# nikola3794/normal-clustering-nerf

Measured on AMD Instinct MI355X. Metric: training rays/sec (+ samples/sec), higher is better.
Workload: dtype fp32 (march/composite/losses); fp16-operand MFMA with fp32 accumulate in the field MLP; 1 GPU; configs[1]+[2]: full training step, 8192 rays/GPU, normal clustering on; rays_per_gpu=8192, global_batch=8192, grid=128, max_samples=1024, parallelism=dp1, grid_update_every_16=True

## Files before the change

### normal-clustering-nerf_amd/csrc/field.hip

```cpp
#include <algorithm>
#include <type_traits>
#include <cstring>
#include "common.h"
#include "../../include/ncnerf.h"

namespace ncn {

typedef float float4_t __attribute__((ext_vector_type(4)));
typedef short short4_t __attribute__((ext_vector_type(4)));

template <typename T> struct Mfma;
template <> struct Mfma<_Float16> {
    static constexpr bool f16 = true;
    typedef _Float16 v4 __attribute__((ext_vector_type(4)));
    typedef _Float16 v8 __attribute__((ext_vector_type(8)));
    static __device__ __forceinline__ float4_t k32(v8 a, v8 b, float4_t c) {
        return __builtin_amdgcn_mfma_f32_16x16x32_f16(a, b, c, 0, 0, 0);
    }
    static __device__ __forceinline__ float4_t k16(v4 a, v4 b, float4_t c) {
        return __builtin_amdgcn_mfma_f32_16x16x16f16(a, b, c, 0, 0, 0);
    }
};
template <> struct Mfma<__bf16> {
    static constexpr bool f16 = false;
// ... 47 lines not shown
constexpr int B_L5 = 0;
constexpr int B_L2 = 4;
constexpr int N_FRAG16 = 8;
constexpr int PACKED_HALVES = N_FRAG32 * 512 + N_FRAG16 * 256;
static_assert(PACKED_HALVES == NCN_FIELD_PACKED_HALVES, "packed size");

constexpr int W1_OFF = 0, W2_OFF = W1_OFF + 64 * 32, W3_OFF = W2_OFF + 16 * 64, W4_OFF = W3_OFF + 64 * 32,
              W5_OFF = W4_OFF + 64 * 64, W_TOTAL = W5_OFF + 16 * 64;
static_assert(W_TOTAL == NCN_FIELD_NW, "weights size");

__host__ __device__ constexpr int phi(int g, int j) { return j < 4 ? 4 * g + j : 16 + 4 * g + (j - 4); }
__host__ __device__ constexpr int psi(int g, int j) {
    return j < 4 ? 3 + 4 * g + j : ((4 * g + j - 4) < 3 ? (4 * g + j - 4) : 16 + (4 * g + j - 4));
}

__host__ __device__ constexpr int frag32_index(int f, int lane, int j) {
    const int g = lane >> 4, r = lane & 15, k = phi(g, j);
    if (f < F_L2) return W1_OFF + (16 * (f - F_L1) + r) * 32 + k;
    if (f < F_L3) return W2_OFF + r * 64 + 32 * (f - F_L2) + k;
    if (f < F_L4) return W3_OFF + (16 * (f - F_L3) + r) * 32 + psi(g, j);
    if (f < F_L5) return W4_OFF + (16 * ((f - F_L4) >> 1) + r) * 64 + 32 * ((f - F_L4) & 1) + k;
    if (f < B_L4) return W5_OFF + r * 64 + 32 * (f - F_L5) + k;
    if (f < B_L3) return W4_OFF + (32 * ((f - B_L4) & 1) + k) * 64 + 16 * ((f - B_L4) >> 1) + r;
    if (f < B_L1) return W3_OFF + (32 * (f - B_L3) + k) * 32 + 3 + r;
    return W1_OFF + (32 * ((f - B_L1) & 1) + k) * 32 + 16 * ((f - B_L1) >> 1) + r;
}
__host__ __device__ constexpr int frag16_index(int f, int lane, int j) {
    const int g = lane >> 4, r = lane & 15, k = 4 * g + j;
    return f < B_L2 ? W5_OFF + k * 64 + 16 * (f - B_L5) + r : W2_OFF + k * 64 + 16 * (f - B_L2) + r;
}
__device__ float frag32_value(const float* __restrict__ W, int f, int lane, int j) { return W[frag32_index(f, lane, j)]; }
__device__ float frag16_value(const float* __restrict__ W, int f, int lane, int j) { return W[frag16_index(f, lane, j)]; }

__global__ void pack_map_kernel(int32_t* __restrict__ src) {
    const int f = blockIdx.x, lane = threadIdx.x;
    if (f < N_FRAG32) {
        for (int j = 0; j < 8; j++) src[(f * 64 + lane) * 8 + j] = frag32_index(f, lane, j);
    } else {
        const int f16 = f - N_FRAG32;
        for (int j = 0; j < 4; j++) src[N_FRAG32 * 512 + (f16 * 64 + lane) * 4 + j] = frag16_index(f16, lane, j);
    }
}

template <typename T>
__global__ void pack_weights_kernel(const float* __restrict__ W, T* __restrict__ out) {
    const int f = blockIdx.x, lane = threadIdx.x;
    if (f < N_FRAG32) {
#pragma unroll
        for (int j = 0; j < 8; j++) out[(f * 64 + lane) * 8 + j] = (T)frag32_value(W, f, lane, j);
    } else {
        const int f16 = f - N_FRAG32;
#pragma unroll
        for (int j = 0; j < 4; j++) out[N_FRAG32 * 512 + (f16 * 64 + lane) * 4 + j] = (T)frag16_value(W, f16, lane, j);
    }
}

struct LevelTable {
    float scale[16];
    uint32_t res[16], params[16], offset[16];
};

__device__ __forceinline__ uint32_t grid_index(uint32_t params, uint32_t res, uint32_t x, uint32_t y, uint32_t z) {
    uint32_t stride = 1, index = 0;
    if (stride <= params) { index += x * stride; stride *= res; }
    if (stride <= params) { index += y * stride; stride *= res; }
    if (stride <= params) { index += z * stride; stride *= res; }
    if (params < stride) index = x ^ (y * 2654435761u) ^ (z * 805459861u);
    if ((params & (params - 1)) == 0) return index & (params - 1);
    return index < params ? index : index % params;
}

struct LevelPos {
    uint32_t px, py, pz;
    float fx, fy, fz;
};
__device__ __forceinline__ LevelPos level_pos(float scale, float x, float y, float z) {
    LevelPos p;
    float a = fmaf(scale, x, 0.5f), b = fmaf(scale, y, 0.5f), c = fmaf(scale, z, 0.5f);
    const float fa = floorf(a), fb = floorf(b), fc = floorf(c);
    p.px = (uint32_t)(int)fa; p.py = (uint32_t)(int)fb; p.pz = (uint32_t)(int)fc;
    p.fx = a - fa; p.fy = b - fb; p.fz = c - fc;
    return p;
}

__device__ __forceinline__ float2 encode_level(const float2* __restrict__ tab, const LevelTable& L, int l, float x,
                                               float y, float z) {
    const LevelPos p = level_pos(L.scale[l], x, y, z);
    const uint32_t params = L.params[l], res = L.res[l], off = L.offset[l];
    uint32_t e[8];
    if ((uint64_t)res * res * res <= params) {
        const uint32_t b0 = p.px + res * p.py + res * res * p.pz;
#pragma unroll
        for (int c = 0; c < 8; c++) {
            const uint32_t i = b0 + (c & 1) + ((c >> 1) & 1) * res + ((c >> 2) & 1) * res * res;
            e[c] = i < params ? i : i % params;
        }
    } else {
        const uint32_t hy0 = p.py * 2654435761u, hy1 = (p.py + 1) * 2654435761u;
        const uint32_t hz0 = p.pz * 805459861u, hz1 = (p.pz + 1) * 805459861u;
        const uint32_t mask = params - 1;
#pragma unroll
        for (int c = 0; c < 8; c++) e[c] = ((p.px + (c & 1)) ^ ((c & 2) ? hy1 : hy0) ^ ((c & 4) ? hz1 : hz0)) & mask;
    }
    float2 v[8];
#pragma unroll
    for (int c = 0; c < 8; c++) v[c] = tab[off + e[c]];
    const float wx[2] = {1.0f - p.fx, p.fx}, wy[2] = {1.0f - p.fy, p.fy}, wz[2] = {1.0f - p.fz, p.fz};
    float2 acc = make_float2(0.f, 0.f);
#pragma unroll
    for (int c = 0; c < 8; c++) {
        const float w = (wx[c & 1] * wy[(c >> 1) & 1]) * wz[c >> 2];
        acc.x = fmaf(w, v[c].x, acc.x);
        acc.y = fmaf(w, v[c].y, acc.y);
    }
    return acc;
}

template <int CTRL>
__device__ __forceinline__ float dppf(float v) {
    return __int_as_float(__builtin_amdgcn_update_dpp(0, __float_as_int(v), CTRL, 0xF, 0xF, false));
}
template <int CTRL>
__device__ __forceinline__ int dppi(int v) {
    return __builtin_amdgcn_update_dpp(0, v, CTRL, 0xF, 0xF, false);
}
constexpr int DPP_ROW_SL(int k) { return 0x100 + k; }
constexpr int DPP_ROW_SR(int k) { return 0x110 + k; }

template <int K>
__device__ __forceinline__ void run_sum(float& v, const int (&link)[4]) {
    const float t = dppf<DPP_ROW_SL(1 << K)>(v);
    if (link[K]) v += t;
}

template <typename T>
struct Frags {
    typedef typename Mfma<T>::v4 v4;
    typedef typename Mfma<T>::v8 v8;
    const v8* f32;
    const v4* f16;
    __device__ __forceinline__ v8 a32(int f, int lane) const { return f32[f * 64 + lane]; }
    __device__ __forceinline__ v4 a16(int f, int lane) const { return f16[f * 64 + lane]; }
};
template <typename T>
struct FragsSigma : Frags<T> {
    __device__ __forceinline__ typename Mfma<T>::v8 a32(int f, int lane) const {
        return this->f32[(f >= B_L1 ? f - (B_L1 - F_L3) : f) * 64 + lane];
    }
    __device__ __forceinline__ typename Mfma<T>::v4 a16(int f, int lane) const {
        return this->f16[(f - B_L2) * 64 + lane];
    }
};
constexpr int N_SIG32 = F_L3 + 4, N_SIG16 = 4;

template <typename T>
struct FwdState {
    typedef typename Mfma<T>::v4 v4;
    v4 x2[4];
    float4_t h;
    v4 x3h, x3d;
    v4 x4[4];
    v4 x5[4];
    float4_t out;
};

template <typename T, typename FR>
__device__ __forceinline__ void mlp_sigma(const FR& F, int lane, typename Mfma<T>::v8 e, FwdState<T>& st) {
    typedef Mfma<T> M;
    typedef typename M::v8 v8;
#pragma unroll
    for (int t = 0; t < 4; t++) st.x2[t] = relu4<T>(M::k32(F.a32(F_L1 + t, lane), e, zero4()));
    float4_t h = M::k32(F.a32(F_L2, lane), cat8<v8>(st.x2[0], st.x2[1]), zero4());
    st.h = M::k32(F.a32(F_L2 + 1, lane), cat8<v8>(st.x2[2], st.x2[3]), h);
}

template <typename T>
__device__ __forceinline__ void mlp_rgb(const Frags<T>& F, int lane, float dnx, float dny, float dnz, FwdState<T>& st) {
    typedef Mfma<T> M;
    typedef typename M::v8 v8;
    const int g = lane >> 4;
    st.x3h = cvt4<T>(st.h);
    st.x3d = cvt4<T>(float4_t{g == 0 ? dnx : 1.f, g == 0 ? dny : 1.f, g == 0 ? dnz : 1.f, 1.f});
    const v8 b3 = cat8<v8>(st.x3h, st.x3d);
#pragma unroll
    for (int t = 0; t < 4; t++) st.x4[t] = relu4<T>(M::k32(F.a32(F_L3 + t, lane), b3, zero4()));
    const v8 b4a = cat8<v8>(st.x4[0], st.x4[1]), b4b = cat8<v8>(st.x4[2], st.x4[3]);
#pragma unroll
    for (int t = 0; t < 4; t++)
        st.x5[t] = relu4<T>(M::k32(F.a32(F_L4 + 2 * t + 1, lane), b4b, M::k32(F.a32(F_L4 + 2 * t, lane), b4a, zero4())));
    const float4_t o = M::k32(F.a32(F_L5, lane), cat8<v8>(st.x5[0], st.x5[1]), zero4());
    st.out = M::k32(F.a32(F_L5 + 1, lane), cat8<v8>(st.x5[2], st.x5[3]), o);
}

__device__ __forceinline__ float sigmoidf_(float x) { return 1.0f / (1.0f + __expf(-x)); }

__device__ __forceinline__ void load_levels(LevelTable& Ls, const LevelTable& La) {
    if (threadIdx.x < 16) {
        const int l = threadIdx.x;
        Ls.scale[l] = La.scale[l];
        Ls.res[l] = La.res[l];
        Ls.params[l] = La.params[l];
        Ls.offset[l] = La.offset[l];
    }
}

constexpr int SORT_W = 4096, SORT_THREADS = 1024;
__device__ __forceinline__ uint32_t sort_spread10(uint32_t v) {
    v &= 0x3FFu;
    v = (v | (v << 16)) & 0x030000FFu;
    v = (v | (v << 8)) & 0x0300F00Fu;
    v = (v | (v << 4)) & 0x030C30C3u;
    v = (v | (v << 2)) & 0x09249249u;
    return v;
}
__device__ __forceinline__ uint32_t sort_q10(float v, float mn, float inv) {
    const float q = (v - mn) * inv * 1024.0f;
    return (uint32_t)(int)fminf(fmaxf(q, 0.0f), 1023.0f);
}
__global__ __launch_bounds__(SORT_THREADS) void sort_windows_kernel(const float* __restrict__ xyzs, int64_t n,
                                                                    const int32_t* __restrict__ n_dev, float mn,
                                                                    float inv, int32_t* __restrict__ order) {
    __shared__ unsigned long long k[SORT_W];
    if (n_dev) n = min<int64_t>(n, *n_dev);
    const int64_t base = (int64_t)blockIdx.x * SORT_W;
    if (base >= n) return;
    const int cnt = (int)min<int64_t>(SORT_W, n - base);
    for (int i = threadIdx.x; i < SORT_W; i += SORT_THREADS) {
        unsigned long long key = ~0ull;
        if (i < cnt) {
            const float* x = xyzs + 3 * (base + i);
            const uint32_t m = sort_spread10(sort_q10(x[0], mn, inv)) | (sort_spread10(sort_q10(x[1], mn, inv)) << 1) |
                               (sort_spread10(sort_q10(x[2], mn, inv)) << 2);
            key = ((unsigned long long)m << 12) | (unsigned long long)i;
        }
        k[i] = key;
    }
    __syncthreads();
    for (int size = 2; size <= SORT_W; size <<= 1) {
        for (int stride = size >> 1; stride > 0; stride >>= 1) {
            for (int t = threadIdx.x; t < SORT_W / 2; t += SORT_THREADS) {
                const int lo = 2 * t - (t & (stride - 1)), hi = lo + stride;
                const bool up = (lo & size) == 0;
                const unsigned long long a = k[lo], b = k[hi];
                if ((a > b) == up) { k[lo] = b; k[hi] = a; }
            }
            __syncthreads();
        }
    }
    for (int i = threadIdx.x; i < cnt; i += SORT_THREADS) order[base + i] = (int32_t)(base + (int64_t)(k[i] & 0xFFFull));
}

template <typename T, bool DENSITY>
__global__ __launch_bounds__(256) __attribute__((amdgpu_waves_per_eu(4))) void field_fwd_kernel(const float* __restrict__ xyzs, const float* __restrict__ dirs,
                                                        int64_t n, const int32_t* __restrict__ n_dev,
                                                        const float2* __restrict__ table, LevelTable Lt,
                                                        float xyz_min, float xyz_extent,
                                                        const typename Mfma<T>::v8* __restrict__ wpacked, int mode,
                                                        float* __restrict__ sigmas, float* __restrict__ rgbs,
                                                        typename Mfma<T>::v8* __restrict__ enc_cache,
                                                        const int32_t* __restrict__ order) {
    typedef typename Mfma<T>::v8 v8;
    __shared__ v8 Fs[N_FWD32 * 64];
    __shared__ LevelTable L;
    const int64_t n16 = (n + 15) & ~(int64_t)15;
    if (n_dev) n = min<int64_t>(n, *n_dev);
    for (int i = threadIdx.x; i < N_FWD32 * 64; i += 256) Fs[i] = wpacked[i];
    load_levels(L, Lt);
    __syncthreads();
    const int lane = threadIdx.x & 63, g = lane >> 4, r = lane & 15;
    const int64_t n_groups = (n + 15) / 16;
    const int64_t wave0 = (int64_t)blockIdx.x * 4 + (threadIdx.x >> 6);
    const int64_t n_waves = (int64_t)gridDim.x * 4;
    for (int64_t grp = wave0; grp < n_groups; grp += n_waves) {
        Frags<T> F;
        F.f32 = Fs + opaque_zero();
        F.f16 = nullptr;
        const int64_t pos = grp * 16 + r;
        const bool valid = pos < n;
        const int64_t s = valid && order ? (int64_t)order[pos] : pos;
        v8 e;
        if constexpr (DENSITY) {
            typedef T t2 __attribute__((ext_vector_type(2)));
            const t2* el = (const t2*)enc_cache + pos;
            const t2 a0 = el[(2 * g) * n16], a1 = el[(2 * g + 1) * n16];
            const t2 b0 = el[(8 + 2 * g) * n16], b1 = el[(9 + 2 * g) * n16];
            e = v8{a0[0], a0[1], a1[0], a1[1], b0[0], b0[1], b1[0], b1[1]};
        } else {
            float x = 0.f, y = 0.f, z = 0.f;
            if (valid) {
                x = (xyzs[3 * s] - xyz_min) / xyz_extent;
                y = (xyzs[3 * s + 1] - xyz_min) / xyz_extent;
                z = (xyzs[3 * s + 2] - xyz_min) / xyz_extent;
            }
            const float2 e00 = encode_level(table, L, 2 * g, x, y, z);
            const float2 e01 = encode_level(table, L, 2 * g + 1, x, y, z);
            asm volatile("; encode: levels 8+ after 0-7 %1 %2" : "+v"(x) : "v"(e00.x), "v"(e01.x));
            const float2 e10 = encode_level(table, L, 8 + 2 * g, x, y, z);
            const float2 e11 = encode_level(table, L, 9 + 2 * g, x, y, z);
            e = v8{(T)e00.x, (T)e00.y, (T)e01.x, (T)e01.y, (T)e10.x, (T)e10.y, (T)e11.x, (T)e11.y};
            if (enc_cache) enc_cache[grp * 64 + lane] = e;
        }
        FwdState<T> st;
        mlp_sigma<T>(F, lane, e, st);
        if (g == 0 && valid) sigmas[s] = __expf(st.h[0]);
        if (DENSITY || mode != 0) continue;
        float dx = 0.f, dy = 0.f, dz = 0.f;
// ... 102 lines not shown
}

__device__ __forceinline__ float lmax_upd(float m, float a, float b) {
    return (isfinite(a) && isfinite(b)) ? fmaxf(m, fmaxf(fabsf(a), fabsf(b))) : INFINITY;
}
template <int PART> constexpr int x_count() { return PART == BWD_SIGMA ? N_XFRAG - XA2 : N_XFRAG; }
template <int PART> constexpr int x_origin() { return PART == BWD_SIGMA ? XA2 : 0; }

template <typename T>
struct DinCtx {
    const T* w3d;
    const int32_t* order;
    float* out;
};
template <typename T, int PART, bool DIN = false, typename FR>
__device__ __forceinline__ void bwd_group(const FR& F, uint16_t* Xw, const BwdIn<T>& cur, int64_t grp,
                                          int64_t n, int64_t n_stride, int lane, float* __restrict__ dE_out,
                                          float (&lm)[4], float inv_S, typename Mfma<T>::v4* __restrict__ stq,
                                          float* __restrict__ sth0, const DinCtx<T>* din = nullptr) {
    typedef Mfma<T> M;
    typedef typename M::v4 v4;
    typedef typename M::v8 v8;
    const int g = lane >> 4, r = lane & 15;
    const int64_t s = grp * 16 + r;
    const bool valid = s < n;
    FwdState<T> st;
    mlp_sigma<T>(F, lane, cur.e, st);
    float4_t dh;
    if constexpr ((PART & BWD_RGB) != 0) {
    float dx = cur.dx, dy = cur.dy, dz = cur.dz;
    if (valid) {
        const float nrm = sqrtf(dx * dx + dy * dy + dz * dz);
        dx /= nrm; dy /= nrm; dz /= nrm;
    }
    mlp_rgb<T>(F, lane, dx, dy, dz, st);
    float4_t dy5 = zero4();
    if (g == 0) {
        const float s0 = sigmoidf_(st.out[0]), s1 = sigmoidf_(st.out[1]), s2 = sigmoidf_(st.out[2]);
        dy5[0] = cur.dr0 * s0 * (1.f - s0);
        dy5[1] = cur.dr1 * s1 * (1.f - s1);
        dy5[2] = cur.dr2 * s2 * (1.f - s2);
    }
    const v4 dy5h = cvt4<T>(dy5);
    x_put(Xw + XA5 * 256, lane, dy5h);
#pragma unroll
    for (int b = 0; b < 4; b++) x_put(Xw + (XB5 + b) * 256, lane, st.x5[b]);
    v4 dD4[4];
#pragma unroll
    for (int t = 0; t < 4; t++) dD4[t] = relu_mask4<T>(M::k16(F.a16(B_L5 + t, lane), dy5h, zero4()), st.x5[t]);
#pragma unroll
    for (int t = 0; t < 4; t++) {
        x_put(Xw + (XA4 + t) * 256, lane, dD4[t]);
        x_put(Xw + (XB4 + t) * 256, lane, st.x4[t]);
    }
    const v8 d4a = cat8<v8>(dD4[0], dD4[1]), d4b = cat8<v8>(dD4[2], dD4[3]);
    v4 dD3[4];
#pragma unroll
    for (int t = 0; t < 4; t++)
        dD3[t] = relu_mask4<T>(M::k32(F.a32(B_L4 + 2 * t + 1, lane), d4b, M::k32(F.a32(B_L4 + 2 * t, lane), d4a, zero4())),
                                st.x4[t]);
#pragma unroll
    for (int t = 0; t < 4; t++) x_put(Xw + (XA3 + t) * 256, lane, dD3[t]);
    x_put(Xw + XB3D * 256, lane, st.x3d);
    x_put(Xw + XB3H * 256, lane, st.x3h);
    if constexpr (DIN) {
        float gi[3] = {0.f, 0.f, 0.f};
#pragma unroll
        for (int k = 0; k < 3; k++)
#pragma unroll
            for (int t = 0; t < 4; t++) {
                const v4 w = *(const v4*)(din->w3d + k * 64 + 16 * t + 4 * g);
#pragma unroll
                for (int i = 0; i < 4; i++) gi[k] = fmaf((float)w[i], (float)dD3[t][i], gi[k]);
            }
#pragma unroll
        for (int k = 0; k < 3; k++) {
            gi[k] += __shfl_xor(gi[k], 16);
            gi[k] += __shfl_xor(gi[k], 32);
        }
        if (g == 0 && valid) {
#pragma unroll
            for (int k = 0; k < 3; k++) gi[k] = (float)(T)gi[k] * inv_S;
            const float nrm = sqrtf(cur.dx * cur.dx + cur.dy * cur.dy + cur.dz * cur.dz);
            const float nx = cur.dx / nrm, ny = cur.dy / nrm, nz = cur.dz / nrm;
            const float ng = nx * gi[0] + ny * gi[1] + nz * gi[2];
            float* o = din->out + 3 * (din->order ? (int64_t)din->order[s] : s);
            o[0] = (gi[0] - nx * ng) / nrm;
            o[1] = (gi[1] - ny * ng) / nrm;
            o[2] = (gi[2] - nz * ng) / nrm;
        }
    }
    dh = M::k32(F.a32(B_L3, lane), cat8<v8>(dD3[0], dD3[1]), zero4());
    dh = M::k32(F.a32(B_L3 + 1, lane), cat8<v8>(dD3[2], dD3[3]), dh);
    if constexpr (PART == BWD_RGB) {
        stq[grp * 64 + lane] = cvt4<T>(dh);
        if (g == 0) sth0[grp * 16 + r] = dh[0];
        return;
    }
    }
    v4 dhh;
    const float tex = __expf(fminf(fmaxf(st.h[0], -15.f), 15.f));
    if constexpr (PART == BWD_SIGMA) {
        dhh = cur.dq;
        if (g == 0) dhh[0] = (T)fmaf(cur.dsig, tex, cur.h0);
    } else {
        dhh = cvt4<T>(dh);
        if (g == 0) dhh[0] = (T)fmaf(cur.dsig, tex, dh[0]);
    }
    constexpr int XO = x_origin<PART>();
    x_put(Xw + (XA2 - XO) * 256, lane, dhh);
#pragma unroll
    for (int b = 0; b < 4; b++) x_put(Xw + (XB2 - XO + b) * 256, lane, st.x2[b]);
    v4 dD1[4];
#pragma unroll
    for (int t = 0; t < 4; t++) dD1[t] = relu_mask4<T>(M::k16(F.a16(B_L2 + t, lane), dhh, zero4()), st.x2[t]);
#pragma unroll
    for (int t = 0; t < 4; t++) x_put(Xw + (XA1 - XO + t) * 256, lane, dD1[t]);
    const v4 e0 = v4{cur.e[0], cur.e[1], cur.e[2], cur.e[3]}, e1 = v4{cur.e[4], cur.e[5], cur.e[6], cur.e[7]};
    x_put(Xw + (XB1 - XO) * 256, lane, e0);
    x_put(Xw + (XB1 - XO + 1) * 256, lane, e1);
    const v8 d1a = cat8<v8>(dD1[0], dD1[1]), d1b = cat8<v8>(dD1[2], dD1[3]);
    float4_t dE[2];
#pragma unroll
    for (int t = 0; t < 2; t++)
        dE[t] = M::k32(F.a32(B_L1 + 2 * t + 1, lane), d1b, M::k32(F.a32(B_L1 + 2 * t, lane), d1a, zero4()));
    typedef T t2 __attribute__((ext_vector_type(2)));
    const t2 q[4] = {t2{(T)dE[0][0], (T)dE[0][1]}, t2{(T)dE[0][2], (T)dE[0][3]}, t2{(T)dE[1][0], (T)dE[1][1]},
                     t2{(T)dE[1][2], (T)dE[1][3]}};
#pragma unroll
    for (int j = 0; j < 4; j++) lm[j] = lmax_upd(lm[j], (float)q[j][0] * inv_S, (float)q[j][1] * inv_S);
    if (valid) {
        t2* o = (t2*)dE_out;
        o[(int64_t)(2 * g) * n_stride + s] = q[0];
        o[(int64_t)(2 * g + 1) * n_stride + s] = q[1];
        o[(int64_t)(8 + 2 * g) * n_stride + s] = q[2];
        o[(int64_t)(9 + 2 * g) * n_stride + s] = q[3];
    }
}

template <typename T, int NX = N_XFRAG, int XO = 0>
__device__ __forceinline__ typename Mfma<T>::v8 x_pair(const uint16_t* X, int q, int ng, int tile, int lane) {
    typedef typename Mfma<T>::v4 v4;
    const v4 a = x_get<v4>(X + (q * NX + tile - XO) * 256, lane);
    const v4 b = q + 1 < ng ? x_get<v4>(X + ((q + 1) * NX + tile - XO) * 256, lane) : v4{0, 0, 0, 0};
    return cat8<typename Mfma<T>::v8>(a, b);
}
template <typename T, int PART>
__device__ __forceinline__ void bwd_dw(const uint16_t* X, int ng, int wid, int lane, float4_t (&acc)[5]) {
    typedef Mfma<T> M;
    typedef typename M::v8 v8;
    constexpr bool RGB = (PART & BWD_RGB) != 0, SIG = (PART & BWD_SIGMA) != 0;
    if constexpr (PART == BWD_SIGMA) {
        constexpr int NX = x_count<PART>(), XO = x_origin<PART>();
        for (int q = 0; q < ng; q += 2) {
            acc[0] = M::k32(x_pair<T, NX, XO>(X, q, ng, XA1 + (wid >> 1), lane),
                            x_pair<T, NX, XO>(X, q, ng, XB1 + (wid & 1), lane), acc[0]);
            if (wid < 4)
                acc[1] = M::k32(x_pair<T, NX, XO>(X, q, ng, XA2, lane), x_pair<T, NX, XO>(X, q, ng, XB2 + wid, lane),
                                acc[1]);
        }
        return;
    }
    if constexpr (PART == BWD_RGB) {
        for (int q = 0; q < ng; q += 2) {
            if (wid < 4) {
                const v8 A4 = x_pair<T>(X, q, ng, XA4 + wid, lane);
#pragma unroll
                for (int b = 0; b < 4; b++) acc[b] = M::k32(A4, x_pair<T>(X, q, ng, XB4 + b, lane), acc[b]);
            } else {
                const v8 A3 = x_pair<T>(X, q, ng, XA3 + wid - 4, lane);
                acc[0] = M::k32(A3, x_pair<T>(X, q, ng, XB3D, lane), acc[0]);
                acc[1] = M::k32(A3, x_pair<T>(X, q, ng, XB3H, lane), acc[1]);
                acc[4] = M::k32(x_pair<T>(X, q, ng, XA5, lane), x_pair<T>(X, q, ng, XB5 + wid - 4, lane), acc[4]);
            }
        }
        return;
    }
    for (int q = 0; q < ng; q += 2) {
        if (wid < 4) {
            if constexpr (RGB) {
                const v8 A4 = x_pair<T>(X, q, ng, XA4 + wid, lane);
#pragma unroll
                for (int b = 0; b < 4; b++) acc[b] = M::k32(A4, x_pair<T>(X, q, ng, XB4 + b, lane), acc[b]);
                acc[4] = M::k32(x_pair<T>(X, q, ng, XA5, lane), x_pair<T>(X, q, ng, XB5 + wid, lane), acc[4]);
            }
        } else if (wid < 6) {
            if constexpr (RGB) {
                const v8 Bd = x_pair<T>(X, q, ng, XB3D, lane), Bh = x_pair<T>(X, q, ng, XB3H, lane);
#pragma unroll
                for (int aa = 0; aa < 2; aa++) {
                    const v8 A3 = x_pair<T>(X, q, ng, XA3 + 2 * (wid - 4) + aa, lane);
                    acc[2 * aa] = M::k32(A3, Bd, acc[2 * aa]);
                    acc[2 * aa + 1] = M::k32(A3, Bh, acc[2 * aa + 1]);
                }
            }
            if constexpr (SIG)
                acc[4] = M::k32(x_pair<T>(X, q, ng, XA2, lane), x_pair<T>(X, q, ng, XB2 + wid - 4, lane), acc[4]);
        } else {
            if constexpr (SIG) {
                const v8 B0 = x_pair<T>(X, q, ng, XB1, lane), B1 = x_pair<T>(X, q, ng, XB1 + 1, lane);
#pragma unroll
                for (int aa = 0; aa < 2; aa++) {
                    const v8 A1 = x_pair<T>(X, q, ng, XA1 + 2 * (wid - 6) + aa, lane);
                    acc[2 * aa] = M::k32(A1, B0, acc[2 * aa]);
                    acc[2 * aa + 1] = M::k32(A1, B1, acc[2 * aa + 1]);
                }
                acc[4] = M::k32(x_pair<T>(X, q, ng, XA2, lane), x_pair<T>(X, q, ng, XB2 + wid - 4, lane), acc[4]);
            }
        }
    }
}

template <int PART>
__device__ __forceinline__ void bwd_store_dw(float* __restrict__ out, int wid, int lane, float4_t (&acc)[5], float inv_S) {
    constexpr bool RGB = (PART & BWD_RGB) != 0, SIG = (PART & BWD_SIGMA) != 0;
    const int g = lane >> 4, r = lane & 15;
#pragma unroll
    for (int t = 0; t < 5; t++)
#pragma unroll
        for (int i = 0; i < 4; i++) acc[t][i] *= inv_S;
    if constexpr (PART == BWD_SIGMA) {
#pragma unroll
        for (int i = 0; i < 4; i++) {
            const int row = 4 * g + i;
            out[W1_OFF + (16 * (wid >> 1) + row) * 32 + 16 * (wid & 1) + r] = acc[0][i];
            if (wid < 4) out[W2_OFF + row * 64 + 16 * wid + r] = acc[1][i];
        }
        return;
    }
    if constexpr (PART == BWD_RGB) {
#pragma unroll
        for (int i = 0; i < 4; i++) {
            const int row = 4 * g + i;
            if (wid < 4) {
#pragma unroll
                for (int b = 0; b < 4; b++) out[W4_OFF + (16 * wid + row) * 64 + 16 * b + r] = acc[b][i];
            } else {
                const int orow = 16 * (wid - 4) + row;
                out[W3_OFF + orow * 32 + (r < 3 ? r : 16 + r)] = acc[0][i];
                out[W3_OFF + orow * 32 + 3 + r] = acc[1][i];
                out[W5_OFF + row * 64 + 16 * (wid - 4) + r] = acc[4][i];
            }
        }
        return;
    }
#pragma unroll
    for (int i = 0; i < 4; i++) {
        const int row = 4 * g + i;
        if (wid < 4) {
            if constexpr (RGB) {
#pragma unroll
                for (int b = 0; b < 4; b++) out[W4_OFF + (16 * wid + row) * 64 + 16 * b + r] = acc[b][i];
                out[W5_OFF + row * 64 + 16 * wid + r] = acc[4][i];
            }
        } else if (wid < 6) {
            if constexpr (RGB) {
#pragma unroll
                for (int aa = 0; aa < 2; aa++) {
                    const int orow = 16 * (2 * (wid - 4) + aa) + row;
                    out[W3_OFF + orow * 32 + (r < 3 ? r : 16 + r)] = acc[2 * aa][i];
                    out[W3_OFF + orow * 32 + 3 + r] = acc[2 * aa + 1][i];
                }
            }
            if constexpr (SIG) out[W2_OFF + row * 64 + 16 * (wid - 4) + r] = acc[4][i];
        } else {
            if constexpr (SIG) {
#pragma unroll
                for (int aa = 0; aa < 2; aa++) {
                    const int orow = 16 * (2 * (wid - 6) + aa) + row;
                    out[W1_OFF + orow * 32 + r] = acc[2 * aa][i];
                    out[W1_OFF + orow * 32 + 16 + r] = acc[2 * aa + 1][i];
                }
                out[W2_OFF + row * 64 + 16 * (wid - 4) + r] = acc[4][i];
            }
        }
    }
}

__host__ __device__ inline int bwd_blocks_of(int64_t n) {
    const int64_t groups = (n + 15) / 16;
    const int64_t b = (groups + 31) / 32;
    return (int)(b < 1 ? 1 : (b > 256 ? 256 : b));
}

template <typename T, int PART = BWD_ALL, bool DIN = false>
__global__ __launch_bounds__(BWD_THREADS) void field_bwd_kernel(
    const float* __restrict__ dirs, int64_t n, const int32_t* __restrict__ n_dev, const uint16_t* __restrict__ wpacked,
    const typename Mfma<T>::v8* __restrict__ enc_cache, const float* __restrict__ dL_dsig,
    const float* __restrict__ dL_drgb, const float* __restrict__ loss_scale, float* __restrict__ dE_out,
    float* __restrict__ slab, float* __restrict__ level_max, const int32_t* __restrict__ order,
    const float* __restrict__ dL_dsig2 = nullptr, float* __restrict__ stash = nullptr,
    const float* __restrict__ xyzs = nullptr, const float* __restrict__ w_master = nullptr,
    float* __restrict__ dL_ddirs = nullptr) {
    static_assert(!DIN || PART == BWD_ALL, "the direction gradient leaves the one-pass form only");
    typedef typename Mfma<T>::v4 v4;
    const float S = loss_scale ? *loss_scale * (Mfma<T>::f16 ? NCN_TCNN_LOSS_SCALE : 1.f) : 1.f, inv_S = 1.f / S;
    typedef typename Mfma<T>::v8 v8;
    const int64_t n_stride = (n + 3) & ~(int64_t)3;
    float* const dE_pairs = dE_out ? dE_out + DE_HEADER_FLOATS : nullptr;
    if (PART != BWD_RGB && dE_out && blockIdx.x == 0 && threadIdx.x < SC_QUEUE_WORDS) {
        if (threadIdx.x == 0) {
            dE_out[0] = inv_S;
            dE_out[1] = Mfma<T>::f16 ? 0.f : 1.f;
        }
        ((unsigned*)(dE_out + de_queue_offset(n_stride)))[threadIdx.x] = 0u;
    }
    const float* pos_src = ((PART & DE_POS_PART) != 0 && dE_out && !order) ? xyzs : nullptr;
    float* const pos_out = pos_src ? dE_out + DE_HEADER_FLOATS + 16 * n_stride : nullptr;
    const int64_t pos_stride = sc_perm_stride(n_stride);
    if ((PART & DE_POS_PART) != 0 && dE_out && blockIdx.x == 0 && threadIdx.x == 0)
        dE_out[DE_POS_FLAG] = pos_out ? (float)((1 << DE_POS_MLP_CLASSES) - 1) : 0.f;
    const int lm_rows = bwd_blocks_of(n);
    v4* stq = (v4*)stash;
    float* sth0 = stash ? stash + ((n + 15) / 16) * 128 : nullptr;
    const int64_t n_cap = n;
    if (n_dev) n = min<int64_t>(n, *n_dev);
    constexpr bool SIGONLY = PART == BWD_SIGMA;
    constexpr int NF32 = SIGONLY ? N_SIG32 : N_FRAG32, NF16 = SIGONLY ? N_SIG16 : N_FRAG16, NX = x_count<PART>();
    __shared__ v8 F32s[NF32 * 64];
    __shared__ v4 F16s[NF16 * 64];
    __shared__ __attribute__((aligned(16))) uint16_t X[BWD_WAVES * NX * 256];
    {
        const v8* w32 = (const v8*)wpacked;
        const v4* w16 = (const v4*)(wpacked + N_FRAG32 * 512);
        for (int i = threadIdx.x; i < NF32 * 64; i += BWD_THREADS) {
            const int f = i >> 6;
            F32s[i] = w32[(SIGONLY && f >= F_L3 ? f + (B_L1 - F_L3) : f) * 64 + (i & 63)];
        }
        for (int i = threadIdx.x; i < NF16 * 64; i += BWD_THREADS) F16s[i] = w16[(SIGONLY ? B_L2 * 64 : 0) + i];
    }
    if constexpr (PART == BWD_RGB) {
        if (blockIdx.x == 0 && level_max)
            for (int i = threadIdx.x; i < lm_rows * 16; i += BWD_THREADS) level_max[i] = 0.f;
    }
    DinCtx<T> din = {nullptr, order, dL_ddirs};
    if constexpr (DIN) {
        __shared__ __attribute__((aligned(16))) T W3d[3 * 64];
        for (int i = threadIdx.x; i < 3 * 64; i += BWD_THREADS) W3d[i] = (T)w_master[W3_OFF + (i & 63) * 32 + (i >> 6)];
        din.w3d = W3d;
        for (int64_t i = 3 * n + (int64_t)blockIdx.x * BWD_THREADS + threadIdx.x; i < 3 * n_cap;
             i += (int64_t)gridDim.x * BWD_THREADS)
            dL_ddirs[i] = 0.f;
    }
    __syncthreads();
    const int lane = threadIdx.x & 63, wid = threadIdx.x >> 6;
    float4_t acc[5];
#pragma unroll
    for (int t = 0; t < 5; t++) acc[t] = zero4();
    float lm[4] = {0.f, 0.f, 0.f, 0.f};
    const int64_t n_groups = (n + 15) / 16;
    const int64_t stride = (int64_t)gridDim.x * BWD_WAVES;
    int64_t base = (int64_t)blockIdx.x * BWD_WAVES;
    BwdIn<T> nxt;
    if (base + wid < n_groups)
        bwd_load<T, PART>(nxt, base + wid, n, lane, enc_cache, dirs, dL_dsig, dL_dsig2, dL_drgb, stq, sth0, order, S,
                          pos_src);
    for (; base < n_groups; base += stride) {
        const int64_t grp = base + wid;
        const int ng = (int)min<int64_t>(BWD_WAVES, n_groups - base);
        const BwdIn<T> cur = nxt;
        if (grp + stride < n_groups)
            bwd_load<T, PART>(nxt, grp + stride, n, lane, enc_cache, dirs, dL_dsig, dL_dsig2, dL_drgb, stq, sth0, order,
                              S, pos_src);
        if (grp < n_groups) {
            if ((PART & DE_POS_PART) != 0 && pos_out && (lane >> 4) < DE_POS_MLP_CLASSES && grp * 16 + (lane & 15) < n) {
                const int cls = lane >> 4;
                float* po = pos_out + cls * 3 * pos_stride + 3 * sc_perm(grp * 16 + (lane & 15), cls);
                po[0] = cur.px; po[1] = cur.py; po[2] = cur.pz;
            }
            typename std::conditional<SIGONLY, FragsSigma<T>, Frags<T>>::type F;
            const int z = opaque_zero();
            F.f32 = F32s + z;
            F.f16 = F16s + z;
            bwd_group<T, PART, DIN>(F, X + wid * NX * 256, cur, grp, n, n_stride, lane, dE_pairs, lm, inv_S, stq, sth0,
                                    &din);
        }
        lds_barrier();
        if constexpr (DIN) {
            bwd_dw<T, PART>(X, __builtin_amdgcn_readfirstlane(ng), __builtin_amdgcn_readfirstlane(wid), lane, acc);
        } else
            bwd_dw<T, PART>(X, ng, wid, lane, acc);
        lds_barrier();
    }
    bwd_store_dw<PART>(slab + (int64_t)blockIdx.x * NCN_FIELD_NW, wid, lane, acc, inv_S);
    if constexpr (PART == BWD_RGB) return;
#pragma unroll
    for (int i = 0; i < 4; i++) {
        float m = lm[i];
        m = fmaxf(m, dppf<0x128>(m));
        m = fmaxf(m, dppf<0x124>(m));
        m = fmaxf(m, dppf<0x122>(m));
        m = fmaxf(m, dppf<0x121>(m));
        lm[i] = m;
    }
    __shared__ float lmw[BWD_WAVES][16];
    if ((lane & 15) == 0) {
        const int g = lane >> 4;
        lmw[wid][2 * g] = lm[0];
        lmw[wid][2 * g + 1] = lm[1];
        lmw[wid][8 + 2 * g] = lm[2];
        lmw[wid][9 + 2 * g] = lm[3];
    }
    __syncthreads();
    if (threadIdx.x < 16) {
        float m = 0.f;
#pragma unroll
        for (int w = 0; w < BWD_WAVES; w++) m = fmaxf(m, lmw[w][threadIdx.x]);
        if constexpr (PART == BWD_SIGMA)
            atomicMax((unsigned*)&level_max[(blockIdx.x % lm_rows) * 16 + threadIdx.x], __float_as_uint(m));
        else
            level_max[blockIdx.x * 16 + threadIdx.x] = m;
    }
    if (PART == BWD_ALL && blockIdx.x == 0)
        for (int i = (int)gridDim.x * 16 + threadIdx.x; i < lm_rows * 16; i += BWD_THREADS) level_max[i] = 0.f;
}

constexpr int WRED_CHUNK = 16;
__global__ void reduce_wgrad_kernel(const float* __restrict__ slab, int nb_sigma, int nb_rgb, float* __restrict__ gw) {
    const int i = blockIdx.x * 256 + threadIdx.x;
    if (i >= NCN_FIELD_NW) return;
    const int nb = i < W3_OFF ? nb_sigma : nb_rgb;
    const int b0 = blockIdx.y * WRED_CHUNK, b1 = min(nb, b0 + WRED_CHUNK);
    if (b0 >= b1) return;
    float s = 0.f;
    for (int b = b0; b < b1; b++) s += slab[(int64_t)b * NCN_FIELD_NW + i];
    atomicAdd(gw + i, s);
}

constexpr int SC_THREADS = 1024;
constexpr int SC_WAVES = SC_THREADS / 64;
constexpr int SC_WAYS = 4;
constexpr int SC_SLOT_BYTES = 4 + 8 + 8 + 2;
constexpr int SC_SETS_DIR = 1536;
constexpr int SC_CELL_HI = 10;
constexpr int SC_CELL_VALS = 16;
constexpr int SC_SETS_CELL = 160;
constexpr int SC_QUEUE = 64;
constexpr int SC_CELL_TABLE_BYTES = SC_SETS_CELL * SC_WAYS * (4 + SC_CELL_VALS * 8 + 2);
constexpr int SC_QUEUE_BYTES = SC_WAVES * SC_QUEUE * (4 + SC_CELL_VALS * 4);
constexpr int sc_max(int a, int b) { return a > b ? a : b; }
constexpr int SC_ARENA = sc_max(SC_CELL_TABLE_BYTES + SC_QUEUE_BYTES, SC_SETS_DIR * SC_WAYS * SC_SLOT_BYTES);
static_assert(SC_CELL_TABLE_BYTES % 16 == 0, "run queues 16-B aligned");
constexpr uint32_t SC_EMPTY = 0xFFFFFFFFu;
constexpr int SC_BATCH = 2;
__host__ __device__ constexpr int sc_fine_c(int l) { return l < 15 ? 4 : 2; }
#ifndef NCN_SC_C_CELL
#define NCN_SC_C_CELL 4
#endif
constexpr int SC_C_CELL = NCN_SC_C_CELL;

__device__ __forceinline__ uint32_t sc_set(uint32_t e, uint32_t sets) { return __umulhi(e * 0x9E3779B1u, sets); }

__device__ __forceinline__ long long sc_fix(float v, int k) {
    const double magic = 6755399441055744.0;
    const double y = fma((double)v, __longlong_as_double((long long)(1023 + k) << 52), magic);
    return __double_as_longlong(y) - __double_as_longlong(magic);
}

struct ScShared {
    uint32_t* keys;
    long long *valx, *valy;
    uint16_t* used;
    float4* qval;
    uint32_t* qkey;
    uint32_t sets;
    int slots;
    int* fill;
    int* grab;
};
enum { SC_MODE_DIR = 0, SC_MODE_CELL = 1 };
__device__ __forceinline__ ScShared sc_layout(char* arena, int* fill, int mode) {
    ScShared sh;
    sh.sets = mode == SC_MODE_CELL ? SC_SETS_CELL : SC_SETS_DIR;
    sh.slots = (int)sh.sets * SC_WAYS;
    sh.valx = (long long*)arena;
    sh.valy = mode == SC_MODE_CELL ? sh.valx + (SC_CELL_VALS - 1) * sh.slots : sh.valx + sh.slots;
    sh.keys = (uint32_t*)(sh.valy + sh.slots);
    sh.used = (uint16_t*)(sh.keys + sh.slots);
    sh.qval = (float4*)(arena + SC_CELL_TABLE_BYTES);
    sh.qkey = (uint32_t*)(sh.qval + SC_WAVES * SC_QUEUE * 4);
    sh.fill = fill;
    return sh;
}

struct ScLevel {
    float scale;
    uint32_t res, params, off;
    bool dense, direct;
    int k;
};

__device__ __forceinline__ void sc_corner_entries(const ScLevel& L, uint32_t px, uint32_t py, uint32_t pz,
                                                  uint32_t (&e)[8]) {
    if (L.dense) {
        const uint32_t b0 = px + L.res * py + L.res * L.res * pz;
#pragma unroll
        for (int c = 0; c < 8; c++) {
            e[c] = b0 + (c & 1) + ((c >> 1) & 1) * L.res + ((c >> 2) & 1) * L.res * L.res;
            e[c] = e[c] < L.params ? e[c] : e[c] % L.params;
        }
    } else {
        const uint32_t hy0 = py * 2654435761u, hy1 = (py + 1) * 2654435761u;
        const uint32_t hz0 = pz * 805459861u, hz1 = (pz + 1) * 805459861u;
#pragma unroll
        for (int c = 0; c < 8; c++)
            e[c] = ((px + (c & 1)) ^ ((c & 2) ? hy1 : hy0) ^ ((c & 4) ? hz1 : hz0)) & (L.params - 1);
    }
}

__device__ __forceinline__ void sc_add(ScShared& sh, int lane, uint32_t px, uint32_t py, uint32_t pz,
                                       const float (&v)[16], const ScLevel& L, float* __restrict__ grad) {
    uint32_t e[8];
    sc_corner_entries(L, px, py, pz, e);
    if (L.direct) {
#pragma unroll
        for (int c = 0; c < 8; c++) {
            if (v[2 * c] != 0.f || v[2 * c + 1] != 0.f) {
                atomicAdd(grad + 2 * (size_t)(L.off + e[c]), v[2 * c]);
                atomicAdd(grad + 2 * (size_t)(L.off + e[c]) + 1, v[2 * c + 1]);
            }
        }
        return;
    }
    uint32_t newmask = 0;
    int slot[8];
#pragma unroll
    for (int c0 = 0; c0 < 8; c0 += SC_BATCH) {
        uint4 kk[SC_BATCH];
        int p0[SC_BATCH];
#pragma unroll
        for (int b = 0; b < SC_BATCH; b++) {
            p0[b] = SC_WAYS * sc_set(e[c0 + b], sh.sets);
            kk[b] = *(const uint4*)&sh.keys[p0[b]];
        }
        int sl[SC_BATCH];
        bool vc[SC_BATCH], miss = false;
#pragma unroll
        for (int b = 0; b < SC_BATCH; b++) {
            const uint32_t k = e[c0 + b];
            vc[b] = (v[2 * (c0 + b)] != 0.f) | (v[2 * (c0 + b) + 1] != 0.f);
            sl[b] = kk[b].x == k ? p0[b] : kk[b].y == k ? p0[b] + 1 : kk[b].z == k ? p0[b] + 2
                  : kk[b].w == k ? p0[b] + 3 : -1;
            miss |= vc[b] && sl[b] < 0;
        }
        if (__ballot(miss)) {
#pragma unroll
            for (int b = 0; b < SC_BATCH; b++) {
                if (vc[b] && sl[b] < 0) {
                    const uint32_t k = e[c0 + b];
#pragma unroll
                    for (int attempt = 0; attempt < 2 && sl[b] < 0; attempt++) {
                        if (attempt) {
                            asm volatile("" ::: "memory");
                            kk[b] = *(const uint4*)&sh.keys[p0[b]];
                        }
                        sl[b] = kk[b].x == k ? p0[b] : kk[b].y == k ? p0[b] + 1 : kk[b].z == k ? p0[b] + 2
                              : kk[b].w == k ? p0[b] + 3 : -1;
                        if (sl[b] >= 0) break;
                        const int cl = kk[b].x == SC_EMPTY ? p0[b] : kk[b].y == SC_EMPTY ? p0[b] + 1
                                     : kk[b].z == SC_EMPTY ? p0[b] + 2 : kk[b].w == SC_EMPTY ? p0[b] + 3 : -1;
                        if (cl < 0) break;
                        const uint32_t got = atomicCAS(&sh.keys[cl], SC_EMPTY, k);
                        if (got == SC_EMPTY) { sl[b] = cl; newmask |= 1u << (c0 + b); }
                        else if (got == k) sl[b] = cl;
                    }
                }
            }
// ... 923 lines not shown
    NCN_LAUNCH_CHECK("ncn_field_bwd_mlp");
    return 0;
}

int ncn_field_bwd_mlp_din(const float* xyzs, const float* dirs, int64_t n, const int32_t* n_dev, const int32_t* order,
                          const uint16_t* weights_packed, int precision, const uint16_t* enc_cache,
                          const float* dL_dsigmas, const float* dL_drgbs, const float* loss_scale, float* slab,
                          float* dE_ws, float* level_max, const float* w_master, float* dL_ddirs, void* stream) {
    if (n <= 0) return 0;
    NCN_REQUIRE(precision == NCN_PREC_F16 || precision == NCN_PREC_BF16, hipErrorInvalidValue,
                "ncn_field_bwd_mlp_din: precision must be NCN_PREC_F16 or NCN_PREC_BF16");
    NCN_REQUIRE(dirs != nullptr, hipErrorInvalidValue,
                "ncn_field_bwd_mlp_din: no direction gradient without dirs (density mode)");
    NCN_REQUIRE(w_master != nullptr && dL_ddirs != nullptr, hipErrorInvalidValue,
                "ncn_field_bwd_mlp_din: w_master and dL_ddirs required");
    NCN_REQUIRE(((uintptr_t)dE_ws & 15) == 0 && ((uintptr_t)enc_cache & 15) == 0 && ((uintptr_t)weights_packed & 15) == 0,
                hipErrorInvalidValue, "ncn_field_bwd_mlp_din: dE_ws / enc_cache / weights_packed must be 16-byte aligned");
    NCN_REQUIRE(level_max != nullptr, hipErrorInvalidValue, "ncn_field_bwd_mlp_din: level_max workspace required");
    NCN_REQUIRE(((uintptr_t)xyzs & 15) == 0, hipErrorInvalidValue, "ncn_field_bwd_mlp_din: xyzs must be 16-byte aligned");
    const int nb = ncn_field_bwd_blocks(n);
    const hipStream_t st = (hipStream_t)stream;
    if (precision == NCN_PREC_F16)
        hipLaunchKernelGGL((field_bwd_kernel<_Float16, BWD_ALL, true>), dim3(nb), dim3(BWD_THREADS), 0, st, dirs, n, n_dev,
                           weights_packed, (const Mfma<_Float16>::v8*)enc_cache, dL_dsigmas, dL_drgbs, loss_scale, dE_ws,
                           slab, level_max, order, (const float*)nullptr, (float*)nullptr, xyzs, w_master, dL_ddirs);
    else
        hipLaunchKernelGGL((field_bwd_kernel<__bf16, BWD_ALL, true>), dim3(nb), dim3(BWD_THREADS), 0, st, dirs, n, n_dev,
                           weights_packed, (const Mfma<__bf16>::v8*)enc_cache, dL_dsigmas, dL_drgbs, loss_scale, dE_ws,
                           slab, level_max, order, (const float*)nullptr, (float*)nullptr, xyzs, w_master, dL_ddirs);
    NCN_LAUNCH_CHECK("ncn_field_bwd_mlp_din");
    return 0;
}

int ncn_field_bwd_dx(const float* xyzs, int64_t n, const int32_t* n_dev, const int32_t* order, const float* table,
                     const uint32_t* levels, float xyz_min, float xyz_extent, const float* dE_ws, float* dL_dxyzs,
                     void* stream) {
    if (n <= 0) return 0;
    NCN_REQUIRE(xyzs && table && levels && dE_ws && dL_dxyzs, hipErrorInvalidValue,
                "ncn_field_bwd_dx: xyzs, table, levels, dE_ws and dL_dxyzs required");
    NCN_REQUIRE(xyz_extent > 0.f, hipErrorInvalidValue, "ncn_field_bwd_dx: xyz_extent must be positive");
    NCN_REQUIRE(((uintptr_t)table & 7) == 0 && ((uintptr_t)dE_ws & 15) == 0, hipErrorInvalidValue,
                "ncn_field_bwd_dx: table 8-byte, dE_ws 16-byte aligned");
    const LevelTable Lt = make_table(levels);
    hipLaunchKernelGGL(field_bwd_dx_kernel, dim3(fwd_grid(n)), dim3(256), 0, (hipStream_t)stream, xyzs, n, n_dev, order,
                       (const float2*)table, Lt, xyz_min, xyz_extent, dE_ws, dL_dxyzs);
    NCN_LAUNCH_CHECK("ncn_field_bwd_dx");
    return 0;
}

int64_t ncn_field_bwd_stash_floats(int64_t n) { return n > 0 ? 144 * ((n + 15) / 16) : 0; }

int ncn_field_bwd_part_blocks(int64_t n, int part) {
    const int nb = ncn_field_bwd_blocks(n);
    return part == 2 ? std::min(512, 2 * nb) : nb;
}

int ncn_field_bwd_mlp_part(const float* xyzs, const float* dirs, int64_t n, const int32_t* n_dev, const int32_t* order,
                           const uint16_t* weights_packed, int precision, const uint16_t* enc_cache,
                           const float* dL_dsigmas, const float* dL_dsigmas2, const float* dL_drgbs,
                           const float* loss_scale, int part, int n_blocks, float* slab, float* dE_ws,
                           float* level_max, float* dh_stash, void* stream) {
    if (n <= 0) return 0;
    NCN_REQUIRE(precision == NCN_PREC_F16 || precision == NCN_PREC_BF16, hipErrorInvalidValue,
                "ncn_field_bwd_mlp_part: precision must be NCN_PREC_F16 or NCN_PREC_BF16");
    NCN_REQUIRE(part == 1 || part == 2 || part == 3, hipErrorInvalidValue,
                "ncn_field_bwd_mlp_part: part must be 1 (rgb), 2 (sigma) or 3 (both)");
    NCN_REQUIRE(((uintptr_t)dE_ws & 15) == 0 && ((uintptr_t)enc_cache & 15) == 0 &&
                    ((uintptr_t)weights_packed & 15) == 0 && ((uintptr_t)dh_stash & 15) == 0,
                hipErrorInvalidValue, "ncn_field_bwd_mlp_part: dE_ws / enc_cache / weights_packed / dh_stash must be 16-byte aligned");
    NCN_REQUIRE(level_max != nullptr, hipErrorInvalidValue, "ncn_field_bwd_mlp_part: level_max workspace required");
    NCN_REQUIRE(part == 3 || dh_stash != nullptr, hipErrorInvalidValue, "ncn_field_bwd_mlp_part: dh_stash required for a split pass");
    const int nb = n_blocks > 0 ? std::min(n_blocks, ncn_field_bwd_part_blocks(n, part))
                                : ncn_field_bwd_part_blocks(n, part);
    const hipStream_t st = (hipStream_t)stream;
    if (part == 1)
        launch_bwd_part<1>(precision, nb, st, xyzs, dirs, n, n_dev, weights_packed, enc_cache, dL_dsigmas, dL_drgbs,
                           loss_scale, dE_ws, slab, level_max, order, dL_dsigmas2, dh_stash);
    else if (part == 2)
        launch_bwd_part<2>(precision, nb, st, xyzs, dirs, n, n_dev, weights_packed, enc_cache, dL_dsigmas, dL_drgbs,
                           loss_scale, dE_ws, slab, level_max, order, dL_dsigmas2, dh_stash);
    else
        launch_bwd_part<3>(precision, nb, st, xyzs, dirs, n, n_dev, weights_packed, enc_cache, dL_dsigmas, dL_drgbs,
                           loss_scale, dE_ws, slab, level_max, order, dL_dsigmas2, dh_stash);
    NCN_LAUNCH_CHECK("ncn_field_bwd_mlp_part");
    return 0;
}

int ncn_field_scatter_wgrad(const float* xyzs, int64_t n, const int32_t* n_dev, const int32_t* order,
                            const uint32_t* levels, float xyz_min, float xyz_extent, const float* dE_ws,
                            const float* level_max, int level_lo, int level_hi, int max_blocks, float* grad_table,
                            const float* slab, int n_blocks_sigma, int n_blocks_rgb, float* grad_w, void* stream) {
    if (n <= 0 || level_hi <= level_lo) return slab ? ncn_field_reduce_wgrad_parts(slab, n_blocks_sigma, n_blocks_rgb,
                                                                                   grad_w, stream) : 0;
    NCN_REQUIRE(0 <= level_lo && level_hi <= 16, hipErrorInvalidValue, "ncn_field_scatter: levels must lie in [0, 16)");
    NCN_REQUIRE(((uintptr_t)dE_ws & 15) == 0 && ((uintptr_t)xyzs & 15) == 0, hipErrorInvalidValue,
                "ncn_field_scatter: dE_ws and xyzs must be 16-byte aligned");
    NCN_REQUIRE(!slab || grad_w, hipErrorInvalidValue, "ncn_field_scatter_wgrad: grad_w required with a slab");
    const LevelTable Lt = make_table(levels);
    int grid = scatter_grid(n);
    if (max_blocks > 0) grid = std::min(grid, max_blocks * (1024 / SC_THREADS));
    hipLaunchKernelGGL(field_scatter_kernel, dim3(grid), dim3(SC_THREADS), 0, (hipStream_t)stream, xyzs, n, n_dev, Lt,
                       xyz_min, xyz_extent, dE_ws, grad_table, level_max, ncn_field_bwd_blocks(n),
                       level_lo, level_hi, order, slab, n_blocks_sigma, n_blocks_rgb, grad_w,
                       (unsigned*)const_cast<float*>(dE_ws + de_queue_offset((n + 3) & ~(int64_t)3)) + 2 * level_lo);
    NCN_LAUNCH_CHECK("ncn_field_scatter");
    return 0;
}

int ncn_field_scatter_positions(const float* xyzs, int64_t n, const int32_t* n_dev, float* dE_ws, void* stream) {
    if (n <= 0) return 0;
    NCN_REQUIRE(((uintptr_t)dE_ws & 15) == 0 && ((uintptr_t)xyzs & 15) == 0, hipErrorInvalidValue,
                "ncn_field_scatter_positions: dE_ws and xyzs must be 16-byte aligned");
    const int64_t e_stride = (n + 3) & ~(int64_t)3;
    const int pgrid = (int)std::max<int64_t>(1, std::min<int64_t>(1024, cdiv(cdiv(n, 4), 256)));
    hipLaunchKernelGGL(sc_perm_positions_kernel, dim3(pgrid), dim3(256), 0, (hipStream_t)stream, xyzs, n, n_dev,
                       (1 << SC_N_CLASSES) - 1, dE_ws + DE_HEADER_FLOATS + 16 * e_stride, dE_ws + DE_POS_FLAG,
                       (float)((1 << SC_N_CLASSES) - 1));
    NCN_LAUNCH_CHECK("ncn_field_scatter_positions");
    return 0;
}

int ncn_field_scatter(const float* xyzs, int64_t n, const int32_t* n_dev, const int32_t* order,
                      const uint32_t* levels, float xyz_min,
                      float xyz_extent, const float* dE_ws, const float* level_max, int level_lo, int level_hi,
                      int max_blocks, float* grad_table, void* stream) {
    return ncn_field_scatter_wgrad(xyzs, n, n_dev, order, levels, xyz_min, xyz_extent, dE_ws, level_max, level_lo,
                                   level_hi, max_blocks, grad_table, nullptr, 0, 0, nullptr, stream);
}

int ncn_field_bwd(const float* xyzs, const float* dirs, int64_t n, const int32_t* n_dev, const int32_t* order,
                  const uint32_t* levels,
                  float xyz_min, float xyz_extent, const uint16_t* weights_packed, int precision,
                  const uint16_t* enc_cache, const float* dL_dsigmas, const float* dL_drgbs, const float* loss_scale,
                  float* grad_table, float* slab, float* dE_ws, float* level_max, void* stream) {
    if (n <= 0) return 0;
    const int e = ncn_field_bwd_mlp(xyzs, dirs, n, n_dev, order, weights_packed, precision, enc_cache, dL_dsigmas, dL_drgbs,
                                    loss_scale, slab, dE_ws, level_max, stream);
    if (e) return e;
    return ncn_field_scatter(xyzs, n, n_dev, order, levels, xyz_min, xyz_extent, dE_ws, level_max, 0, 16, 0,
                             grad_table, stream);
}


#ifdef NCN_DIAG_SC_TIMES
int ncn_diag_sc_times(unsigned long long* host, int reset) {
    if (reset) {
        static unsigned long long zero[256][10];
        return (int)hipMemcpyToSymbol(HIP_SYMBOL(ncn_sc_times), zero, sizeof(zero));
    }
    return (int)hipMemcpyFromSymbol(host, HIP_SYMBOL(ncn_sc_times), 256 * 10 * sizeof(unsigned long long));
}
#endif

#ifdef NCN_DIAG_SC_SPAN
int ncn_diag_sc_span(unsigned long long* host) {
    return (int)hipMemcpyFromSymbol(host, HIP_SYMBOL(ncn_sc_span), 256 * 20 * sizeof(unsigned long long));
}
#endif

int ncn_field_reduce_wgrad(const float* slab, int n_blocks, float* grad_w, void* stream) {
    if (n_blocks <= 0) return 0;
    hipLaunchKernelGGL(reduce_wgrad_kernel, dim3(cdiv(NCN_FIELD_NW, 256), cdiv(n_blocks, WRED_CHUNK)), dim3(256), 0,
                       (hipStream_t)stream, slab, n_blocks, n_blocks, grad_w);
    NCN_LAUNCH_CHECK("ncn_field_reduce_wgrad");
    return 0;
}

int ncn_field_reduce_wgrad_parts(const float* slab, int n_blocks_sigma, int n_blocks_rgb, float* grad_w,
                                 void* stream) {
    const int nb = std::max(n_blocks_sigma, n_blocks_rgb);
    if (nb <= 0) return 0;
    hipLaunchKernelGGL(reduce_wgrad_kernel, dim3(cdiv(NCN_FIELD_NW, 256), cdiv(nb, WRED_CHUNK)), dim3(256), 0,
                       (hipStream_t)stream, slab, n_blocks_sigma, n_blocks_rgb, grad_w);
    NCN_LAUNCH_CHECK("ncn_field_reduce_wgrad_parts");
    return 0;
}

}
```

Before: 11.46 million rays/s.

## Hold sigma-only backward weight fragments in registers and overlap first load

The sigma-only backward kernel now copies most of its MFMA weight fragments from LDS into registers once per block, instead of reading them from LDS on every group. It issues the first group's input load before the weight staging and barrier, fully unrolls the weight-gradient loop when a block has a full set of groups, and sets a higher minimum waves-per-EU launch bound for the sigma part. Cycle-counter probes are added behind a diagnostic macro that is off by default. The extra register use competes with the occupancy hint and could cause spills.

Result: faster. 11.70 million rays/s (median of 6 runs) (+2.1%).

```diff
diff --git a/normal-clustering-nerf_amd/csrc/field.hip b/normal-clustering-nerf_amd/csrc/field.hip
--- a/normal-clustering-nerf_amd/csrc/field.hip
+++ b/normal-clustering-nerf_amd/csrc/field.hip
@@ -223,6 +223,24 @@
     }
 };
 constexpr int N_SIG32 = F_L3 + 4, N_SIG16 = 4;
+template <typename T>
+struct FragsSigmaReg {
+    typename Mfma<T>::v8 r32[N_SIG32];
+    const typename Mfma<T>::v8* f32;
+    const typename Mfma<T>::v4* f16;
+    __device__ __forceinline__ void load(const FragsSigma<T>& F, int lane) {
+#pragma unroll
+        for (int f = 0; f < N_SIG32; f++)
+            if (f < F_L2 || f >= F_L3) r32[f] = F.f32[f * 64 + lane];
+        f32 = F.f32;
+        f16 = F.f16;
+    }
+    __device__ __forceinline__ typename Mfma<T>::v8 a32(int f, int lane) const {
+        if (f >= F_L2 && f < F_L3) return f32[f * 64 + lane];
+        return r32[f >= B_L1 ? f - (B_L1 - F_L3) : f];
+    }
+    __device__ __forceinline__ typename Mfma<T>::v4 a16(int f, int lane) const { return f16[(f - B_L2) * 64 + lane]; }
+};
 
 template <typename T>
 struct FwdState {
@@ -631,6 +649,17 @@
     constexpr bool RGB = (PART & BWD_RGB) != 0, SIG = (PART & BWD_SIGMA) != 0;
     if constexpr (PART == BWD_SIGMA) {
         constexpr int NX = x_count<PART>(), XO = x_origin<PART>();
+        if (ng == BWD_WAVES) {
+#pragma unroll
+            for (int q = 0; q < BWD_WAVES; q += 2) {
+                acc[0] = M::k32(x_pair<T, NX, XO>(X, q, BWD_WAVES, XA1 + (wid >> 1), lane),
+                                x_pair<T, NX, XO>(X, q, BWD_WAVES, XB1 + (wid & 1), lane), acc[0]);
+                if (wid < 4)
+                    acc[1] = M::k32(x_pair<T, NX, XO>(X, q, BWD_WAVES, XA2, lane),
+                                    x_pair<T, NX, XO>(X, q, BWD_WAVES, XB2 + wid, lane), acc[1]);
+            }
+            return;
+        }
         for (int q = 0; q < ng; q += 2) {
             acc[0] = M::k32(x_pair<T, NX, XO>(X, q, ng, XA1 + (wid >> 1), lane),
                             x_pair<T, NX, XO>(X, q, ng, XB1 + (wid & 1), lane), acc[0]);
@@ -762,8 +791,21 @@
     return (int)(b < 1 ? 1 : (b > 256 ? 256 : b));
 }
 
+#ifdef NCN_DIAG_SIGMA_TIMES
+__device__ unsigned long long ncn_sigma_times[512][10];
+#define SG_TNOW(v) const unsigned long long v = __builtin_readcyclecounter()
+#define SG_TADD(i, a, b) if (PART == BWD_SIGMA && threadIdx.x == 0 && blockIdx.x < 512) ncn_sigma_times[blockIdx.x][i] += (b) - (a)
+#define SG_TREAL(i) if (PART == BWD_SIGMA && threadIdx.x == 0 && blockIdx.x < 512) ncn_sigma_times[blockIdx.x][i] = __builtin_amdgcn_s_memrealtime()
+#define SG_TWAIT() asm volatile("s_waitcnt vmcnt(0)" ::: "memory")
+#else
+#define SG_TNOW(v)
+#define SG_TADD(i, a, b)
+#define SG_TREAL(i)
+#define SG_TWAIT()
+#endif
+
 template <typename T, int PART = BWD_ALL, bool DIN = false>
-__global__ __launch_bounds__(BWD_THREADS) void field_bwd_kernel(
+__global__ __launch_bounds__(BWD_THREADS, PART == BWD_SIGMA ? 4 : 2) void field_bwd_kernel(
     const float* __restrict__ dirs, int64_t n, const int32_t* __restrict__ n_dev, const uint16_t* __restrict__ wpacked,
     const typename Mfma<T>::v8* __restrict__ enc_cache, const float* __restrict__ dL_dsig,
     const float* __restrict__ dL_drgb, const float* __restrict__ loss_scale, float* __restrict__ dE_out,
@@ -799,6 +841,17 @@
     __shared__ v8 F32s[NF32 * 64];
     __shared__ v4 F16s[NF16 * 64];
     __shared__ __attribute__((aligned(16))) uint16_t X[BWD_WAVES * NX * 256];
+    SG_TREAL(6);
+    const int lane = threadIdx.x & 63, wid = threadIdx.x >> 6;
+    const int64_t n_groups = (n + 15) / 16;
+    const int64_t stride = (int64_t)gridDim.x * BWD_WAVES;
+    int64_t base = (int64_t)blockIdx.x * BWD_WAVES;
+    BwdIn<T> nxt;
+    if constexpr (SIGONLY) {
+        if (base + wid < n_groups)
+            bwd_load<T, PART>(nxt, base + wid, n, lane, enc_cache, dirs, dL_dsig, dL_dsig2, dL_drgb, stq, sth0, order, S,
+                              pos_src);
+    }
     {
         const v8* w32 = (const v8*)wpacked;
         const v4* w16 = (const v4*)(wpacked + N_FRAG32 * 512);
@@ -822,22 +875,30 @@
             dL_ddirs[i] = 0.f;
     }
     __syncthreads();
-    const int lane = threadIdx.x & 63, wid = threadIdx.x >> 6;
     float4_t acc[5];
 #pragma unroll
     for (int t = 0; t < 5; t++) acc[t] = zero4();
     float lm[4] = {0.f, 0.f, 0.f, 0.f};
-    const int64_t n_groups = (n + 15) / 16;
-    const int64_t stride = (int64_t)gridDim.x * BWD_WAVES;
-    int64_t base = (int64_t)blockIdx.x * BWD_WAVES;
-    BwdIn<T> nxt;
-    if (base + wid < n_groups)
-        bwd_load<T, PART>(nxt, base + wid, n, lane, enc_cache, dirs, dL_dsig, dL_dsig2, dL_drgb, stq, sth0, order, S,
-                          pos_src);
+    if constexpr (!SIGONLY) {
+        if (base + wid < n_groups)
+            bwd_load<T, PART>(nxt, base + wid, n, lane, enc_cache, dirs, dL_dsig, dL_dsig2, dL_drgb, stq, sth0, order, S,
+                              pos_src);
+    }
+    FragsSigmaReg<T> FR;
+    if constexpr (SIGONLY) {
+        FragsSigma<T> Fl;
+        Fl.f32 = F32s;
+        Fl.f16 = F16s;
+        FR.load(Fl, lane);
+    }
+    SG_TREAL(7);
     for (; base < n_groups; base += stride) {
         const int64_t grp = base + wid;
         const int ng = (int)min<int64_t>(BWD_WAVES, n_groups - base);
         const BwdIn<T> cur = nxt;
+        SG_TNOW(g0);
+        SG_TWAIT();
+        SG_TNOW(g1);
         if (grp + stride < n_groups)
             bwd_load<T, PART>(nxt, grp + stride, n, lane, enc_cache, dirs, dL_dsig, dL_dsig2, dL_drgb, stq, sth0, order,
                               S, pos_src);
@@ -847,20 +908,36 @@
                 float* po = pos_out + cls * 3 * pos_stride + 3 * sc_perm(grp * 16 + (lane & 15), cls);
                 po[0] = cur.px; po[1] = cur.py; po[2] = cur.pz;
             }
-            typename std::conditional<SIGONLY, FragsSigma<T>, Frags<T>>::type F;
-            const int z = opaque_zero();
-            F.f32 = F32s + z;
-            F.f16 = F16s + z;
-            bwd_group<T, PART, DIN>(F, X + wid * NX * 256, cur, grp, n, n_stride, lane, dE_pairs, lm, inv_S, stq, sth0,
-                                    &din);
-        }
+            if constexpr (SIGONLY) {
+                bwd_group<T, PART, DIN>(FR, X + wid * NX * 256, cur, grp, n, n_stride, lane, dE_pairs, lm, inv_S, stq,
+                                        sth0, &din);
+            } else {
+                Frags<T> F;
+                const int z = opaque_zero();
+                F.f32 = F32s + z;
+                F.f16 = F16s + z;
+                bwd_group<T, PART, DIN>(F, X + wid * NX * 256, cur, grp, n, n_stride, lane, dE_pairs, lm, inv_S, stq,
+                                        sth0, &din);
+            }
+        }
+        SG_TNOW(g2);
         lds_barrier();
+        SG_TNOW(g3);
         if constexpr (DIN) {
             bwd_dw<T, PART>(X, __builtin_amdgcn_readfirstlane(ng), __builtin_amdgcn_readfirstlane(wid), lane, acc);
         } else
             bwd_dw<T, PART>(X, ng, wid, lane, acc);
+        SG_TNOW(g4);
         lds_barrier();
-    }
+        SG_TNOW(g5);
+        SG_TADD(0, g0, g1);
+        SG_TADD(1, g1, g2);
+        SG_TADD(2, g2, g3);
+        SG_TADD(3, g3, g4);
+        SG_TADD(4, g4, g5);
+        SG_TADD(5, 0ull, 1ull);
+    }
+    SG_TREAL(8);
     bwd_store_dw<PART>(slab + (int64_t)blockIdx.x * NCN_FIELD_NW, wid, lane, acc, inv_S);
     if constexpr (PART == BWD_RGB) return;
 #pragma unroll
@@ -892,6 +969,7 @@
     }
     if (PART == BWD_ALL && blockIdx.x == 0)
         for (int i = (int)gridDim.x * 16 + threadIdx.x; i < lm_rows * 16; i += BWD_THREADS) level_max[i] = 0.f;
+    SG_TREAL(9);
 }
 
 constexpr int WRED_CHUNK = 16;
@@ -2121,6 +2199,16 @@
 }
 #endif
 
+#ifdef NCN_DIAG_SIGMA_TIMES
+int ncn_diag_sigma_times(unsigned long long* host, int reset) {
+    if (reset) {
+        static unsigned long long zero[512][10];
+        return (int)hipMemcpyToSymbol(HIP_SYMBOL(ncn_sigma_times), zero, sizeof(zero));
+    }
+    return (int)hipMemcpyFromSymbol(host, HIP_SYMBOL(ncn_sigma_times), 512 * 10 * sizeof(unsigned long long));
+}
+#endif
+
 #ifdef NCN_DIAG_SC_SPAN
 int ncn_diag_sc_span(unsigned long long* host) {
     return (int)hipMemcpyFromSymbol(host, HIP_SYMBOL(ncn_sc_span), 256 * 20 * sizeof(unsigned long long));
```
